# ChangUk/RecommenderSystems

Hardware: AMD Instinct MI355X
Metric: RWR seeds/sec + achieved HBM GB/s on 100M-edge bipartite graph, 1/2/4/8 GPUs (higher is better)
Workload: dtype f64

## Files before the change

### recommendersystems_amd/csrc/chain_scan.hip

```cpp
#include "engine.h"
#include "pf.h"

#include <cstdlib>

namespace rwr {

template <int G> struct CsGeom {
    static constexpr int EP = (G == 1) ? 1024 : 4096;
    static constexpr int P = (G >= 16) ? 4 : 1;
    static constexpr int E = EP * P;
    static constexpr int R = EP / 256;
    static constexpr int CH = E / G;
};
__device__ __forceinline__ int cs_pad(int q) { return q + (q >> 4); }
__device__ __forceinline__ double cs_term(const double *termp, const double *zt, const int32_t *srcp, int32_t l, int G)
{
    return zt ? zt[(size_t)srcp[l] * G] : termp[l];
}

__global__ __launch_bounds__(256) void k_cs_links(int nchunks, int CH, const int64_t *__restrict__ in_ptr,
                                                  const int32_t *__restrict__ in_src,
                                                  const int32_t *__restrict__ seeds, int32_t *__restrict__ lnk)
{
    const int slot = blockIdx.y;
// ... 288 lines not shown
{
    const int slot = blockIdx.x, lane = threadIdx.x;
    const int tile = slot / G, k = slot % G;
    const int32_t sd = seeds[slot];
    if (sd < 0) return;
    const size_t base = (size_t)slot * nchunks;
    double s = 0.0;
    unsigned redo = 0;
    if (direct) {
        for (int c = 0; c < nchunks; ++c)
            s = cs_redo_block<G>(s, n, nchunks, c, tile, k, dangling, X, seeds, c1, in_ptr, in_src, evoff, evterm, lnk);
        if (lane == 0) {
            if (sums) sums[slot] = s;
            else Y[(size_t)tile * (size_t)n * G + (size_t)sd * G + k] = s;
            if (zout) { const double rw = c1 * s; zout[(size_t)tile * (size_t)n * G + (size_t)sd * G + k] = rw * w_src[sd]; }
            if (nz_out && s != 0.0)
                atomicOr(&nz_out[(size_t)tile * (((size_t)n + 31) / 32) + ((uint32_t)sd >> 5)], 1u << (sd & 31));
        }
        return;
    }
    double ap, apn = 0.0;
    int32_t ep, epn = 0;
    long long f0, f1, f0n = 0, f1n = 0;
#define CS_LOAD(C, AP, EP, F0, F1)                                   \
    {                                                                \
        const int cc__ = (C) + lane;                                 \
        const bool v__ = cc__ < nchunks;                             \
        const size_t i__ = base + (v__ ? cc__ : nchunks - 1);        \
        AP = v__ ? approx[i__] : 0.0;                                \
        EP = e_pred[i__];                                            \
        F0 = d0[i__];                                                \
        F1 = d1[i__];                                                \
// ... 29 lines not shown
        const int L = __builtin_ctzll(bad);
        if (L > 0 && normal) s = cs_from_m(eb, __shfl(M, L - 1, WAVE));
        s = cs_redo_block<G>(s, n, nchunks, c + L, tile, k, dangling, X, seeds, c1, in_ptr, in_src, evoff, evterm, lnk);
        ++redo;
        done = L + 1;
        if (done >= WAVE || c + done >= nchunks) {
            c += WAVE;
            done = 0;
            ap = apn; ep = epn; f0 = f0n; f1 = f1n;
        }
    }
#undef CS_LOAD
    if (lane == 0) {
        if (sums) sums[slot] = s;
        else Y[(size_t)tile * (size_t)n * G + (size_t)sd * G + k] = s;
        if (nz_out && s != 0.0)
            atomicOr(&nz_out[(size_t)tile * (((size_t)n + 31) / 32) + ((uint32_t)sd >> 5)], 1u << (sd & 31));
        if (redo_count && redo) atomicAdd(redo_count, (unsigned long long)redo);
    }
}

constexpr int CS_PLAIN = 0, CS_SPLIT = 1, CS_EXACT = 2, CS_REDO = 3, CS_SPLIT2 = 4;
#ifdef RWR_EXPERIMENTS
__device__ int cs_carry_dbg = 0;
#endif
constexpr int CS_KIND_SHIFT = 12;
constexpr int CS_SIDE_WORDS = 32;
constexpr int CS_MX_LINKS = 8192;
constexpr int CS_RUN_ADDENDS = 8;
typedef double v2d_t __attribute__((ext_vector_type(2)));

__global__ __launch_bounds__(256, 6) void k_cs_block1(int32_t n, int nchunks, const uint8_t *__restrict__ dangling,
// ... 730 lines not shown
```

### recommendersystems_amd/csrc/common.h

```cpp
#pragma once
#include <hip/hip_runtime.h>
#include <stdint.h>
#include <stdio.h>
#include <string>
#include <vector>

#include "../../include/rwr.h"

namespace rwr {

void set_error(const char *fmt, ...);

#define RWR_HIP(call)                                                                         \
    do {                                                                                      \
        hipError_t e__ = (call);                                                              \
        if (e__ != hipSuccess) {                                                              \
            rwr::set_error("%s failed: %s (%s:%d)", #call, hipGetErrorString(e__), __FILE__,  \
                           __LINE__);                                                         \
            return (e__ == hipErrorOutOfMemory) ? RWR_E_NOMEM : RWR_E_HIP;                    \
        }                                                                                     \
    } while (0)

#define RWR_TRY(call)                  \
    do {                               \
// ... 11 lines not shown

static inline unsigned cdiv(size_t a, size_t b) { return (unsigned)((a + b - 1) / b); }

__host__ __device__ static inline uint64_t f64_orderable(double x)
{
    x = x + 0.0;
    uint64_t u;
    __builtin_memcpy(&u, &x, 8);
    return (u & 0x8000000000000000ull) ? ~u : (u | 0x8000000000000000ull);
}
__host__ __device__ static inline uint64_t i64_orderable(int64_t x)
{
    return (uint64_t)x ^ 0x8000000000000000ull;
}

void *pool_alloc(size_t bytes, size_t *got);
void pool_free(void *p, size_t got);

template <typename T>
struct DevBuf {
    T *p = nullptr;
    size_t count = 0;
    size_t reserved = 0;
    int32_t alloc(size_t n_elems)
    {
        release();
        if (n_elems == 0) n_elems = 1;
        p = (T *)pool_alloc(n_elems * sizeof(T), &reserved);
        if (!p) {
            const hipError_t e = hipGetLastError();
// ... 31 lines not shown
```

### recommendersystems_amd/csrc/iterate.hip

```cpp
#include "engine.h"
#include "step_plan.h"

#include <algorithm>
#include <chrono>
#include <climits>
#include <cstdlib>
#include <new>
#include <type_traits>

namespace rwr {

template <int G, bool VF>
__global__ __launch_bounds__(256) void k_spmm(int32_t n, const int64_t *__restrict__ in_ptr,
                                              const int32_t *__restrict__ in_src,
                                              const double *__restrict__ in_w,
                                              const int32_t *__restrict__ row_order, int32_t nrows,
                                              const double *__restrict__ X, double *__restrict__ Y,
                                              const int32_t *__restrict__ seeds, double c1, int skip_seed_row,
                                              const double *__restrict__ w_src, double *__restrict__ Zout)
{
    constexpr int RPW = WAVE / G;
    constexpr int U = 4;
    const int tile = blockIdx.y;
    const size_t toff = (size_t)tile * (size_t)n * G;
// ... 56 lines not shown
                                                  const int32_t *__restrict__ row_order, int32_t nrows,
                                                  const double *__restrict__ X, double *__restrict__ Y,
                                                  const int32_t *__restrict__ seeds, double c1,
                                                  int skip_seed_row, const uint32_t *__restrict__ nz_in,
                                                  uint32_t *__restrict__ nz_out,
                                                  const uint32_t *__restrict__ act,
                                                  const double *__restrict__ w_src, double *__restrict__ Zout)
{
    static_assert(G >= 8 && G <= 64, "chunked SpMM needs 8 <= G <= 64");
    constexpr int RPW = WAVE / G;
    const int tile = blockIdx.y;
    const size_t toff = (size_t)tile * (size_t)n * G;
    X += toff;
    Y += toff;
    if (VF && Zout) Zout += toff;
    const size_t nzw = ((size_t)n + 31) / 32;
    if (CHECK) nz_in += (size_t)tile * nzw;
    if (WRITE) nz_out += (size_t)tile * nzw;
    if (CHECK && act) act += (size_t)tile * nzw;
    const int lane = threadIdx.x & (WAVE - 1);
    const int sub = lane / G, k = lane % G;
    const int gbase = (lane - k) << 2;
    const int32_t my_seed = skip_seed_row ? seeds[tile * G + k] : -1;
    const int wpb = blockDim.x / WAVE;
    const int64_t nwaves = (int64_t)gridDim.x * wpb;
    for (int64_t rb = ((int64_t)blockIdx.x * wpb + threadIdx.x / WAVE) * RPW; rb < nrows; rb += nwaves * RPW) {
        const int64_t r = rb + sub;
        int32_t j = -1;
        int64_t p = 0, e = 0;
        if (r < nrows) {
            j = row_order[r];
            p = in_ptr[j];
            e = in_ptr[j + 1];
            if (CHECK && act && !((act[(uint32_t)j >> 5] >> (j & 31)) & 1u)) e = p;
        }
        double acc = 0.0;
        while (__any(p < e)) {
            const int64_t left = e - p;
            const int cnt = left > CH ? CH : (left > 0 ? (int)left : 0);
            int32_t my_idx = 0;
            double my_w = 0.0;
            if (k < cnt) {
                my_idx = in_src[p + k];
                if (!VF) my_w = in_w[p + k];
                if (CHECK) {
                    const uint32_t wd = nz_in[(uint32_t)my_idx >> 5];
                    if (!((wd >> (my_idx & 31)) & 1u)) my_idx |= (int32_t)0x80000000;
                }
            }
            const int wlo = __double2loint(my_w), whi = __double2hiint(my_w);
            if (CHECK) {
                const unsigned long long lm = __ballot(k < cnt && my_idx >= 0);
                unsigned long long um = lm;
                if (G < 64) {
#pragma unroll
                    for (int sh = G; sh < 64; sh <<= 1) um |= um >> sh;
                    um &= (1ull << (G & 63)) - 1ull;
                }
                if (__popcll(um) <= 4) {
                    while (um) {
                        const int t = __builtin_ctzll(um);
                        um &= um - 1;
                        const int idx = __builtin_amdgcn_ds_bpermute(gbase + (t << 2), my_idx);
                        if (VF) {
                            if (t < cnt && idx >= 0) acc += X[(size_t)idx * G + k];
                        } else {
                            const int lo = __builtin_amdgcn_ds_bpermute(gbase + (t << 2), wlo);
                            const int hi = __builtin_amdgcn_ds_bpermute(gbase + (t << 2), whi);
                            if (t < cnt && idx >= 0) {
                                const double rw = c1 * X[(size_t)idx * G + k];
                                acc += rw * __hiloint2double(hi, lo);
                            }
                        }
                    }
                    p += cnt;
                    continue;
                }
            }
            double xv[CH], wv[CH];
#pragma unroll
            for (int t = 0; t < CH; ++t) {
                const int idx = __builtin_amdgcn_ds_bpermute(gbase + (t << 2), my_idx);
                if (!VF) {
                    const int lo = __builtin_amdgcn_ds_bpermute(gbase + (t << 2), wlo);
                    const int hi = __builtin_amdgcn_ds_bpermute(gbase + (t << 2), whi);
                    wv[t] = __hiloint2double(hi, lo);
                }
                xv[t] = (t < cnt && idx >= 0) ? X[(size_t)idx * G + k] : 0.0;
            }
#pragma unroll
            for (int t = 0; t < CH; ++t) {
                if (t < cnt) {
                    if (VF) {
                        acc += xv[t];
                    } else {
                        double rw = c1 * xv[t];
                        acc += rw * wv[t];
                    }
                }
            }
            p += cnt;
        }
        if (j >= 0 && j != my_seed) {
            Y[(size_t)j * G + k] = acc;
            if (VF && Zout) { const double rw = c1 * acc; Zout[(size_t)j * G + k] = rw * w_src[j]; }
        }
        if (WRITE) {
            const unsigned long long nzb = __ballot(acc != 0.0);
            const unsigned long long gmask = (G == 64) ? ~0ull : (((1ull << (G & 63)) - 1ull) << (sub * G));
            if (k == 0 && j >= 0 && (nzb & gmask)) atomicOr(&nz_out[(uint32_t)j >> 5], 1u << (j & 31));
        }
    }
}

template <int G, int CH, bool CHECK, bool WRITE, bool VF, bool LIST>
__global__ __launch_bounds__(256) void k_spmm_chunked(int32_t n, const int64_t *__restrict__ in_ptr,
                                                      const int32_t *__restrict__ in_src,
                                                      const double *__restrict__ in_w,
                                                      const int32_t *__restrict__ row_order, int32_t nrows,
                                                      const double *__restrict__ X, double *__restrict__ Y,
                                                      const int32_t *__restrict__ seeds, double c1,
                                                      int skip_seed_row, const uint32_t *__restrict__ nz_in,
                                                      uint32_t *__restrict__ nz_out,
                                                      const uint32_t *__restrict__ act,
                                                      const double *__restrict__ w_src, double *__restrict__ Zout)
// ... 12 lines not shown
                                                       const int32_t *__restrict__ seeds, double c1,
                                                       int skip_seed_row, const uint32_t *__restrict__ nz_in,
                                                       uint32_t *__restrict__ nz_out,
                                                       const double *__restrict__ w_src, double *__restrict__ Zout)
{
    const int tile = blockIdx.y;
    spmm_chunked_body<G, CH, true, true, VF>(n, in_ptr, in_src, in_w, fl_rows + (size_t)tile * (size_t)n, fl_cnt[tile], X, Y,
                                             seeds, c1, skip_seed_row, nz_in, nz_out, nullptr, w_src, Zout);
}

__global__ __launch_bounds__(256) void k_mark_active(int32_t n, const uint32_t *__restrict__ nz, uint32_t *__restrict__ act,
                                                     const int64_t *__restrict__ rowptr, const int32_t *__restrict__ dst,
                                                     const uint8_t *__restrict__ etype, int G, const int32_t *__restrict__ seeds,
                                                     int32_t *__restrict__ fl_rows, int32_t *__restrict__ fl_cnt)
{
    const size_t nzw = ((size_t)n + 31) / 32;
    const int tile = blockIdx.y;
    const int lane = threadIdx.x & (WAVE - 1);
    const size_t wi = (size_t)blockIdx.x * (blockDim.x / WAVE) + threadIdx.x / WAVE;
    uint32_t *a = act + (size_t)tile * nzw;
    int32_t *list = fl_rows ? fl_rows + (size_t)tile * (size_t)n : nullptr;
    if (list && blockIdx.x == 0 && threadIdx.x < (unsigned)G) {
        const int32_t sr = seeds[tile * G + threadIdx.x];
        if (sr >= 0) {
            const uint32_t bit = 1u << (sr & 31);
            if (!(atomicOr(&a[(uint32_t)sr >> 5], bit) & bit)) list[atomicAdd(&fl_cnt[tile], 1)] = sr;
        }
    }
    if (wi >= nzw) return;
    uint32_t w = nz[(size_t)tile * nzw + wi];
    while (w) {
        const int b = __builtin_ctz(w);
        w &= w - 1;
        const int64_t i = (int64_t)wi * 32 + b;
        const int64_t p1 = rowptr[i + 1];
        if (!list) {
            for (int64_t p = rowptr[i] + lane; p < p1; p += WAVE)
                if (etype[p] != RWR_EDGE_UNDEFINED) {
                    const int32_t t = dst[p];
                    atomicOr(&a[(uint32_t)t >> 5], 1u << (t & 31));
                }
            continue;
        }
        for (int64_t p0 = rowptr[i]; p0 < p1; p0 += WAVE) {
            const int64_t p = p0 + lane;
            bool add = false;
            int32_t t = 0;
            if (p < p1 && etype[p] != RWR_EDGE_UNDEFINED) {
                t = dst[p];
// ... 50 lines not shown
            }
            acc += dg[u] ? xv[u] : (xv[u] - rw);
        }
    }
    for (; i < n; ++i) {
        double xi = x[(size_t)i * G];
        double rw = c1 * xi;
        while (nxt == i) {
            acc += rw * in_w[p];
            ++p;
            nxt = (p < e) ? in_src[p] : INT_MAX;
        }
        acc += dangling[i] ? xi : (xi - rw);
    }
    Y[(size_t)tile * (size_t)n * G + (size_t)s * G + k] = acc;
    if (nz_out && acc != 0.0)
        atomicOr(&nz_out[(size_t)tile * (((size_t)n + 31) / 32) + ((uint32_t)s >> 5)], 1u << (s & 31));
}

__global__ void k_gate(const unsigned int *__restrict__ gate, unsigned int expected)
{
    const long long t0 = __builtin_amdgcn_s_memrealtime();
    while (__hip_atomic_load(gate, __ATOMIC_RELAXED, __HIP_MEMORY_SCOPE_AGENT) < expected) {
        if (__builtin_amdgcn_s_memrealtime() - t0 > 100000) break;
        __builtin_amdgcn_s_sleep(32);
    }
}

template <int G, bool VF>
__global__ __launch_bounds__(256) void k_seed_terms(int32_t n, const int64_t *__restrict__ in_ptr,
                                                    const int32_t *__restrict__ in_src,
                                                    const double *__restrict__ in_w, const double *__restrict__ X,
                                                    const int32_t *__restrict__ seeds, double c1,
                                                    const int64_t *__restrict__ evoff, double *__restrict__ evterm,
                                                    const uint32_t *__restrict__ nz)
{
    const int slot = blockIdx.y;
    const int32_t s = seeds[slot];
    if (s < 0) return;
    const int tile = slot / G, k = slot % G;
    const double *x = X + (size_t)tile * (size_t)n * G + k;
    const int64_t p0 = in_ptr[s], deg = in_ptr[s + 1] - p0;
    double *out = evterm + evoff[slot];
    if (nz) nz += (size_t)tile * (((size_t)n + 31) / 32);
    for (int64_t q = (int64_t)blockIdx.x * blockDim.x + threadIdx.x; q < deg; q += (int64_t)gridDim.x * blockDim.x) {
        const int32_t i = in_src[p0 + q];
        if (nz && !((nz[(uint32_t)i >> 5] >> (i & 31)) & 1u)) {
            out[q] = 0.0;
        } else if (VF) {
            out[q] = x[(size_t)i * G];
        } else {
            const double rw = c1 * x[(size_t)i * G];
            out[q] = rw * in_w[p0 + q];
        }
    }
}

template <int G>
__global__ __launch_bounds__(64) void k_seed_chain_sparse(int32_t n, const int64_t *__restrict__ in_ptr,
                                                          const int32_t *__restrict__ in_src,
                                                          const uint8_t *__restrict__ dangling,
                                                          const double *__restrict__ X, double *__restrict__ Y,
                                                          const int32_t *__restrict__ seeds, double c1,
                                                          const int64_t *__restrict__ evoff,
                                                          const double *__restrict__ evterm,
                                                          const uint32_t *__restrict__ nz_x, uint32_t *__restrict__ nz_out,
                                                          unsigned int *__restrict__ gate)
{
    if (threadIdx.x == 0 && gate) __hip_atomic_fetch_add(gate, 1u, __ATOMIC_RELAXED, __HIP_MEMORY_SCOPE_AGENT);
    const int tile = blockIdx.x, lane = threadIdx.x;
    const size_t nzw = ((size_t)n + 31) / 32;
    const uint32_t *bits = nz_x + (size_t)tile * nzw;
    const double *x = X + (size_t)tile * (size_t)n * G;
    const bool consumer = lane < G;
    const int k = lane % G;
    int32_t s = -1;
    int64_t p = 0, e = 0;
    const double *termp = evterm;
    if (consumer) {
        s = seeds[tile * G + k];
        if (s >= 0) {
            p = in_ptr[s];
            e = in_ptr[s + 1];
            termp = evterm + evoff[tile * G + k] - p;
        }
    }
    double acc = 0.0;
    for (size_t w0 = 0; w0 < nzw; w0 += WAVE) {
        const uint32_t word = (w0 + lane < nzw) ? bits[w0 + lane] : 0u;
        unsigned long long mask = __ballot(word != 0u);
        while (mask) {
            const int l = __builtin_ctzll(mask);
            mask &= mask - 1;
            uint32_t wv = (uint32_t)__builtin_amdgcn_readlane((int)word, l);
            while (wv) {
                const int b = __builtin_ctz(wv);
                wv &= wv - 1;
                const int32_t i = (int32_t)((w0 + l) * 32 + b);
                if (consumer && s >= 0) {
                    while (p < e && in_src[p] < i) ++p;
                    while (p < e && in_src[p] == i) { acc += termp[p]; ++p; }
                    const double xi = x[(size_t)i * G + k];
                    const double rw = c1 * xi;
                    acc += dangling[i] ? xi : (xi - rw);
                }
            }
        }
    }
    if (consumer && s >= 0) {
        Y[(size_t)tile * (size_t)n * G + (size_t)s * G + k] = acc;
        if (nz_out && acc != 0.0)
            atomicOr(&nz_out[(size_t)tile * nzw + ((uint32_t)s >> 5)], 1u << (s & 31));
    }
}

constexpr int CH3_NSW = 6;
constexpr int CH3_NST = CH3_NSW * WAVE;
constexpr int CH3_LPT = 16;
constexpr int CH3_CE = CH3_NST * CH3_LPT;
template <int G>
__global__ __launch_bounds__(WAVE + CH3_NST) void k_seed_chain_roles(
    int32_t n, const int64_t *__restrict__ in_ptr, const int32_t *__restrict__ in_src,
    const uint8_t *__restrict__ dangling, const double *__restrict__ X, double *__restrict__ Y,
    const int32_t *__restrict__ seeds, double c1, const int64_t *__restrict__ evoff,
    const double *__restrict__ evterm, uint32_t *__restrict__ nz_out, unsigned int *__restrict__ gate)
{
    if (threadIdx.x == 0 && gate) __hip_atomic_fetch_add(gate, 1u, __ATOMIC_RELAXED, __HIP_MEMORY_SCOPE_AGENT);
// ... 105 lines not shown
        CH3_READ(ra, 0)
#pragma unroll 1
        for (int r0 = 0; r0 + 64 <= CR; r0 += 64) {
            CH3_READ(rb, r0 + 32)
            CH3_FOLD(ra, r0)
            if (r0 + 64 < CR) CH3_READ(ra, r0 + 64)
            CH3_FOLD(rb, r0 + 32)
        }
        if (CR % 64 != 0) CH3_FOLD(ra, CR - 32)
#undef CH3_READ
#undef CH3_FOLD
    }
    __builtin_amdgcn_s_setprio(0);
    if (consumer && s >= 0) {
        Y[(size_t)tile * (size_t)n * G + (size_t)s * G + k] = acc;
        if (nz_out && acc != 0.0)
            atomicOr(&nz_out[(size_t)tile * (((size_t)n + 31) / 32) + ((uint32_t)s >> 5)], 1u << (s & 31));
    }
}

__global__ void k_init_seeds(int32_t n, int ntiles, int G, double *__restrict__ X,
                             const int32_t *__restrict__ seeds, uint32_t *__restrict__ nz,
                             double *__restrict__ Z = nullptr, const double *__restrict__ w_src = nullptr, double c1 = 0.0)
{
    const int q = blockIdx.x * blockDim.x + threadIdx.x;
    if (q >= ntiles * G) return;
    const int32_t s = seeds[q];
    if (s < 0) return;
    const int tile = q / G;
    const size_t row = (size_t)tile * (size_t)n * G + (size_t)s * G;
    const double rw = c1 * (double)n;
    const double zs = Z ? rw * w_src[s] : 0.0;
    for (int kk = 0; kk < G; ++kk) {
        const bool mine = seeds[tile * G + kk] == s;
        X[row + kk] = mine ? (double)n : 0.0;
        if (Z) Z[row + kk] = mine ? zs : 0.0;
    }
    if (nz) atomicOr(&nz[(size_t)tile * (((size_t)n + 31) / 32) + ((uint32_t)s >> 5)], 1u << (s & 31));
}

__global__ __launch_bounds__(64) void k_exclude(int32_t n, int ntiles, int G, const int64_t *__restrict__ rowptr,
                                                const int32_t *__restrict__ dst, const uint8_t *__restrict__ etype,
                                                double *__restrict__ X, const int32_t *__restrict__ seeds)
{
    const int q = blockIdx.x;
    if (q >= ntiles * G) return;
    const int32_t s = seeds[q];
    if (s < 0) return;
    double *x = X + (size_t)(q / G) * (size_t)n * G + (q % G);
    const int64_t p1 = rowptr[s + 1];
    for (int64_t p = rowptr[s] + threadIdx.x; p < p1; p += WAVE)
        if (etype[p] == RWR_EDGE_LIKE) x[(size_t)dst[p] * G] = -1.0;
}
// ... 11 lines not shown
}
__global__ __launch_bounds__(256) void k_make_z(int64_t elems, int G, const double *__restrict__ X, double *__restrict__ Z,
                                                const double *__restrict__ w_src, double c1)
{
    const int64_t q = (int64_t)blockIdx.x * blockDim.x + threadIdx.x;
    if (q >= elems) return;
    const double rw = c1 * X[q];
    Z[q] = rw * w_src[q / G];
}

__global__ __launch_bounds__(256) void k_make_z_nz(int32_t lo, int32_t hi, int G, const double *__restrict__ X, double *__restrict__ Zs,
                                                   const double *__restrict__ w_src, double c1, uint32_t *__restrict__ nz)
{
    const int64_t j = ((int64_t)lo & ~(int64_t)63) + (int64_t)blockIdx.x * blockDim.x + threadIdx.x;
    bool any = false;
    if (j >= lo && j < hi) {
        const double w = w_src[j];
        const size_t at = (size_t)(j - lo) * G;
        for (int k = 0; k < G; ++k) {
            const double xv = X[(size_t)j * G + k];
            const double rw = c1 * xv;
            Zs[at + k] = rw * w;
            any = any || xv != 0.0;
        }
    }
    const unsigned long long m = __ballot(any);
    const int lane = threadIdx.x & (WAVE - 1);
    if (lane == 0 && (uint32_t)m) nz[(uint64_t)j >> 5] = (uint32_t)m;
    if (lane == 32 && (uint32_t)(m >> 32)) nz[(uint64_t)j >> 5] = (uint32_t)(m >> 32);
}


static PlanInput read_plan_knobs()
{
    PlanInput v;
    const char *e;
    if ((e = getenv("RWR_SPMM"))) v.spmm = atoi(e);
    if ((e = RWR_TUNE_ENV("RWR_NZ_ITERS"))) v.nz_iters = atoi(e);
    if ((e = getenv("RWR_ACT_ITERS"))) v.act_iters = atoi(e);
// ... 190 lines not shown
        : g(g_), G(G_), tg(tg_), d_seeds(seeds), d_evoff(evoff), c1(1 - d) ,
          X(g_->X.p), Y(g_->Y.p), Zc(g_->vf ? g_->Z0.p : nullptr), Zn(g_->vf ? g_->Z1.p : nullptr) {}

    int32_t init(bool fresh = true, bool ranks_nonneg = true, bool ranking_only = false)
    {
        const int32_t n = g->n;
        hipStream_t s = g->stream;
        const size_t elems = (size_t)tg * (size_t)n * G;
        PlanInput in = plan_knobs();
        in.n = n; in.nnz = g->nnz; in.nonneg = g->nonneg; in.big_n = spmv_big_n(); in.seed_row_kernel = g->opts.seed_row_kernel;
        in.scan_self = chain_scan_self_contained(G); in.G = G; in.tg = tg; in.c1 = c1;
        in.fresh = fresh; in.ranks_nonneg = ranks_nonneg; in.ranking_only = ranking_only;
        cfg = plan_config(in);
        if (fresh) RWR_HIP(hipMemsetAsync(X, 0, elems * sizeof(double), s));
        if (!fresh && Zc) hipLaunchKernelGGL(k_make_z, dim3(cdiv(elems, 256)), dim3(256), 0, s, (int64_t)elems, G, X, Zc, g->w_src.p, c1);
        const size_t nzw = ((size_t)n + 31) / 32;
        if (cfg.flist && g->fl_rows.ensure((size_t)tg * (size_t)n + (size_t)tg) != RWR_OK) {
            (void)hipGetLastError();
            cfg.flist = false;
        }
        if (fresh && Zc && !cfg.flist) RWR_HIP(hipMemsetAsync(Zc, 0, elems * sizeof(double), s));
        nz_cur = cfg.nz_iters > 0 ? g->d_nz.p : nullptr;
        nz_oth = cfg.nz_iters > 0 ? g->d_nz.p + (size_t)tg * nzw : nullptr;
        if (nz_cur) RWR_HIP(hipMemsetAsync(nz_cur, 0, (size_t)tg * nzw * sizeof(uint32_t), s));
        if (fresh) hipLaunchKernelGGL(k_init_seeds, dim3(cdiv((size_t)tg * G, 64)), dim3(64), 0, s, n, tg, G, X, d_seeds, nz_cur, Zc, g->w_src.p, c1);
        RWR_HIP(hipGetLastError());
        if (cfg.scan) RWR_TRY(chain_scan_prepare(g, G, tg, d_seeds, s));
        if (Zc && G == 1 && tg == 1 && cfg.addends_nonneg) RWR_TRY(sweep_prepare(g));
        if (Zc && cfg.chain_kind == 0 && !cfg.scan) RWR_TRY(ensure_in_w(g));
        return RWR_OK;
    }

    int32_t step(const StepPlan &p, Profile &prof)
    {
        const int32_t n = g->n;
        hipStream_t s = g->stream;
        const size_t nzw = ((size_t)n + 31) / 32;
        constexpr int GATE_SLOTS = 64;
        const uint32_t *nz_in = p.probe ? nz_cur : nullptr;
        uint32_t *nz_out = p.write_bits ? nz_oth : nullptr;
        if (nz_out) RWR_HIP(hipMemsetAsync(nz_out, 0, (size_t)tg * nzw * sizeof(uint32_t), s));
        uint32_t *act = p.mark ? g->d_nz.p + 2 * (size_t)tg * nzw : nullptr;
        const bool listed = p.rows.kind == Rows::Frontier;
        if (act) {
            int32_t *fl_rows = listed ? g->fl_rows.p : nullptr, *fl_cnt = listed ? fl_rows + (size_t)tg * (size_t)n : nullptr;
            RWR_HIP(hipMemsetAsync(act, 0, (size_t)tg * nzw * sizeof(uint32_t), s));
            if (fl_cnt) RWR_HIP(hipMemsetAsync(fl_cnt, 0, (size_t)tg * sizeof(int32_t), s));
            hipLaunchKernelGGL(k_mark_active, dim3(cdiv(nzw, 4), tg), dim3(256), 0, s, n, nz_in, act, g->rowptr.p,
                               g->dst.p, g->etype.p, G, d_seeds, fl_rows, fl_cnt);
        }
        const uint32_t *nz_terms = p.terms_nz ? nz_in : nullptr;
        double *zout = (Zc && p.form_z) ? Zn : nullptr;
        hipStream_t sc = p.chain_side ? g->stream2 : s;
        unsigned int *gate_it = p.gate ? g->d_gate.p + (it % GATE_SLOTS) : nullptr;
        if (p.chain != Chain::None) {
            if (!p.scan()) RWR_DISPATCH_G(G, launch_seed_terms<GG>(g, tg, X, d_seeds, c1, d_evoff, s, Zc, nz_terms));
            if (gate_it) RWR_HIP(hipMemsetAsync(gate_it, 0, sizeof(unsigned int), s));
            if (p.chain_side) { RWR_HIP(hipEventRecord(g->ev_fork, s)); RWR_HIP(hipStreamWaitEvent(sc, g->ev_fork, 0)); }
            if (p.scan() && !(p.chain_self && Zc)) RWR_DISPATCH_G(G, launch_seed_terms<GG>(g, tg, X, d_seeds, c1, d_evoff, sc, Zc, nz_terms));
            hipEvent_t c0; RWR_TRY(prof.record(c0, sc));
            if (p.scan())
                RWR_TRY(chain_scan_step(g, G, tg, X, Y, d_seeds, d_evoff, c1, nz_out, sc, p.chain_self ? Zc : nullptr,
                                        p.chain_self ? zout : nullptr));
// ... 55 lines not shown
    const size_t per_tile = mats * n * (size_t)G * sizeof(double);
    int TG = g->opts.tile_group > 0 ? g->opts.tile_group : (int)(cap / (per_tile ? per_tile : 1));
    if (TG < 1) TG = 1;
    if (TG > ntiles) TG = ntiles;
    if (TG > 65535 / G) TG = 65535 / G;
    if (g->opts.tile_group <= 0 && TG > 192) TG = 192;
    for (;;) {
        int32_t rc = g->X.ensure((size_t)TG * n * G);
        if (rc == RWR_OK) rc = g->Y.ensure((size_t)TG * n * G);
        if (rc == RWR_OK && g->vf) {
            rc = g->Z0.ensure((size_t)TG * n * G);
            if (rc == RWR_OK) rc = g->Z1.ensure((size_t)TG * n * G);
        }
        if (rc == RWR_OK && extra_mats) rc = g->cs_diff.ensure((size_t)TG * n * G);
        if (rc == RWR_OK) rc = g->d_seeds.ensure((size_t)ntiles * G);
        if (rc == RWR_OK) rc = g->d_nz.ensure(3 * (size_t)TG * ((n + 31) / 32));
        if (rc == RWR_OK) rc = g->d_gate.ensure(64);
        if (rc == RWR_OK) break;
        if (rc != RWR_E_NOMEM || TG <= 1 || g->opts.tile_group > 0) return rc;
        (void)hipGetLastError();
        g->X.release(); g->Y.release(); g->Z0.release(); g->Z1.release(); g->d_nz.release();
        if (extra_mats) g->cs_diff.release();
        TG = (TG + 1) / 2;
    }
    *TG_out = TG;
    return RWR_OK;
}

static int32_t upload_seed_slots(rwr_graph *g, const int32_t *seeds, int32_t K, int G, std::vector<int32_t> *slot_k_out,
                                 std::vector<int32_t> *slot_seed_out = nullptr)
{
// ... 558 lines not shown

int32_t part_begin(rwr_graph *g, int32_t lo, int32_t hi, const int32_t *seeds, int32_t K, double d, double *x,
                   int32_t *G_out)
{
    const int32_t n = g->n;
    if (lo < 0 || hi > n || lo > hi) { set_error("rwr_part_begin: bad slab [%d, %d)", lo, hi); return RWR_E_RANGE; }
    if (K < 1 || K > 64) { set_error("rwr_part_begin: K must be 1..64 in row-partitioned mode"); return RWR_E_UNSUPPORTED; }
    for (int32_t k = 0; k < K; ++k)
        if (seeds[k] < 0 || seeds[k] >= n) { set_error("seed %d is outside [0, %d)", seeds[k], n); return RWR_E_RANGE; }
    int G = 1;
    while (G < K) G <<= 1;
    if (g->vf) RWR_TRY(g->Z0.ensure((size_t)(hi - lo > 0 ? hi - lo : 1) * (size_t)G));
    else RWR_TRY(ensure_in_w(g));
    g->part_lo = lo; g->part_hi = hi; g->part_G = G; g->part_K = K; g->part_c1 = 1 - d;
    g->part_steps = 0;
    if (g->vf && g->nonneg && G >= 8) RWR_TRY(g->d_nz.ensure(2 * (((size_t)n + 31) / 32)));
    g->part_seeds.assign((size_t)G, -1);
    for (int32_t k = 0; k < K; ++k) g->part_seeds[k] = seeds[k];
    RWR_TRY(g->d_seeds.ensure(G));
    RWR_TRY(g->d_part.ensure((size_t)RP_GRID * G + G));
    RWR_HIP(hipMemcpy(g->d_seeds.p, g->part_seeds.data(), G * sizeof(int32_t), hipMemcpyHostToDevice));
    hipStream_t s = g->stream;
    RWR_HIP(hipMemsetAsync(x, 0, (size_t)n * G * sizeof(double), s));
    hipLaunchKernelGGL(k_init_seeds, dim3(1), dim3(64), 0, s, n, 1, G, x, g->d_seeds.p, (uint32_t *)nullptr);
    RWR_HIP(hipGetLastError());
    RWR_HIP(hipStreamSynchronize(s));
    if (G_out) *G_out = G;
    return RWR_OK;
}

static int32_t part_spmm(rwr_graph *g, const double *x, double *y, hipStream_t s)
{
    const int G = g->part_G;
    const double c1 = g->part_c1;
    if (g->vf) {
        const int64_t rows = (int64_t)g->part_hi - g->part_lo;
        if (rows > 0 && (!g->Z0.p || g->Z0.count < (size_t)rows * G)) { set_error("rwr_part_step: call rwr_part_begin"); return RWR_E_INVALID; }
        const int64_t elems = rows * G;
        const double *zin = g->Z0.p - (size_t)g->part_lo * G;
        static const int part_act_env = [] { const char *e = RWR_TUNE_ENV("RWR_PART_ACT_STEPS"); return e ? atoi(e) : 2; }();
        static const int part_nz_env = [] { const char *e = RWR_TUNE_ENV("RWR_PART_NZ_STEPS"); return e ? atoi(e) : 4; }();
        const size_t nzw = ((size_t)g->n + 31) / 32;
        const bool frontier = g->part_steps < part_nz_env && g->nonneg && G >= 8 && rows > 0 && g->d_nz.p && g->d_nz.count >= 2 * nzw;
        const bool mark = frontier && g->part_steps < part_act_env;
        ++g->part_steps;
        if (frontier) {
            uint32_t *nz = g->d_nz.p, *act = g->d_nz.p + nzw;
            RWR_HIP(hipMemsetAsync(nz, 0, (mark ? 2 : 1) * nzw * sizeof(uint32_t), s));
            const int64_t first = (int64_t)g->part_lo & ~(int64_t)63;
            hipLaunchKernelGGL(k_make_z_nz, dim3(cdiv((size_t)((int64_t)g->part_hi - first), 256)), dim3(256), 0, s, g->part_lo, g->part_hi, G, x,
                               g->Z0.p, g->w_src.p, c1, nz);
            if (mark) hipLaunchKernelGGL(k_mark_active, dim3(cdiv(nzw, 4), 1), dim3(256), 0, s, g->n, nz, act, g->rowptr.p, g->dst.p, g->etype.p,
                                         0, nullptr, nullptr, nullptr);
            RWR_DISPATCH_G(G, launch_spmm<GG>(g, 1, x, y, g->d_seeds.p, c1, 0, nz, nullptr, s, mark ? act : nullptr, zin, nullptr, false));
            return RWR_OK;
        }
        if (elems > 0)
            hipLaunchKernelGGL(k_make_z, dim3(cdiv((size_t)elems, 256)), dim3(256), 0, s, elems, G, x + (size_t)g->part_lo * G, g->Z0.p,
                               g->w_src.p + g->part_lo, c1);
        RWR_DISPATCH_G(G, launch_spmm<GG>(g, 1, x, y, g->d_seeds.p, c1, 0, nullptr, nullptr, s, nullptr, zin, nullptr, false));
    } else {
        if (!g->in_w.p) { set_error("rwr_part_step: call rwr_part_begin"); return RWR_E_INVALID; }
        RWR_DISPATCH_G(G, launch_spmm<GG>(g, 1, x, y, g->d_seeds.p, c1, 0, nullptr, nullptr, s));
    }
    return RWR_OK;
}

int32_t part_local_step(rwr_graph *g, const double *x, double *y, double *r)
// ... 77 lines not shown
```

### recommendersystems_amd/csrc/step_plan.h

```cpp
#pragma once

#include <cstdint>

namespace rwr {

struct PlanInput {
    int spmm = 1, nz_iters = 4, act_iters = -1, frontier_list = 1, chain = 1;
    int64_t act_min_n = 200000; double scan_work = 10000.0;
    int scan_side = 1, gate = 1, tail_rows = 1;
    bool two_streams = true;
    int32_t n = 0, big_n = 2000000;
    int64_t nnz = 0; bool nonneg = true;
    int seed_row_kernel = 0;
    bool scan_self = false;
    int G = 1, tg = 1;
    double c1 = 0.85;
    bool fresh = true;
    bool ranks_nonneg = true;
    bool ranking_only = false;
};

struct PlanConfig {
    int G = 1, tg = 1; bool fresh = true;
    int nz_iters = 0;
    int act_iters = 0;
    bool flist = false;
    bool addends_nonneg = false;
    bool scan = false;
    int chain_kind = 1;
    bool scan_side = false, scan_self = false;
    bool two_streams = true, gate = true;
    bool tails = false; int tail_depth = 0;
    unsigned need = 0;
};

inline PlanConfig plan_config(const PlanInput &in)
{
    PlanConfig c;
    c.G = in.G, c.tg = in.tg, c.fresh = in.fresh;
    const bool single = in.G == 1 && in.tg == 1;
    c.nz_iters = (in.G >= 8 && in.spmm != 0 && in.nonneg) ? in.nz_iters : 0;
    c.act_iters = in.act_iters >= 0 ? in.act_iters : ((in.nnz / (in.n > 0 ? in.n : 1)) <= 64 ? 2 : 1);
    if (single && in.act_iters < 0 && c.act_iters == 2 && in.n >= in.big_n) c.act_iters = 3;
    if (single && in.spmm != 0 && in.nonneg) c.nz_iters = c.act_iters;
    if (single && in.act_iters < 0 && in.n < in.act_min_n) c.nz_iters = c.act_iters = 0;
    if (!in.fresh) c.nz_iters = c.act_iters = 0;
    c.flist = in.ranking_only && in.fresh && in.frontier_list != 0 && in.G >= 8 && c.nz_iters >= 2 && c.act_iters >= 1;
    c.chain_kind = in.seed_row_kernel == 1 ? 3 : in.seed_row_kernel == 2 ? 2 : in.seed_row_kernel == 3 ? 0 : in.chain;
    const double per_seed = 0.89 * (double)in.nnz / (double)(in.n > 0 ? in.n : 1) + 6.7;
    c.addends_nonneg = in.c1 >= 0.0 && in.c1 <= 1.0 && in.nonneg && in.ranks_nonneg;
    c.scan = c.addends_nonneg && (c.chain_kind == 2 || (c.chain_kind == 1 && (double)in.tg * in.G * per_seed < in.scan_work));
    c.scan_side = in.scan_side != 0 && single && in.two_streams && in.n >= 100000;
    c.scan_self = in.scan_self, c.two_streams = in.two_streams, c.gate = in.gate != 0;
    c.tails = in.ranking_only && in.tail_rows != 0 && !single;
    return c;
}
// ... 53 lines not shown
```

Baseline: 772.7.

## Track nonzero frontier bits per 16-seed line instead of per row

Replaces the one-bit-per-row nonzero bitmap with a multi-bit-per-row bitmap for G>16, one bit per group of 16 seed columns. The SpMM gather then skips X loads for 16-lane groups whose seeds have not yet reached a source row, rather than loading whenever any seed in the tile has. This costs a larger bitmap, extra mask arithmetic in the inner loop, and an index-width limit that disables the frontier path for large n. Frontier consumers (mark_active, sparse chain) collapse the lines back to per-row bits.

```diff
diff --git a/recommendersystems_amd/csrc/chain_scan.hip b/recommendersystems_amd/csrc/chain_scan.hip
--- a/recommendersystems_amd/csrc/chain_scan.hip
+++ b/recommendersystems_amd/csrc/chain_scan.hip
@@ -326,8 +326,7 @@
             if (sums) sums[slot] = s;
             else Y[(size_t)tile * (size_t)n * G + (size_t)sd * G + k] = s;
             if (zout) { const double rw = c1 * s; zout[(size_t)tile * (size_t)n * G + (size_t)sd * G + k] = rw * w_src[sd]; }
-            if (nz_out && s != 0.0)
-                atomicOr(&nz_out[(size_t)tile * (((size_t)n + 31) / 32) + ((uint32_t)sd >> 5)], 1u << (sd & 31));
+            if (nz_out && s != 0.0) nz_set_lines(nz_out + (size_t)tile * nz_words(n, G), sd, G, nz_slot_line(k, G));
         }
         return;
     }
@@ -387,8 +386,7 @@
     if (lane == 0) {
         if (sums) sums[slot] = s;
         else Y[(size_t)tile * (size_t)n * G + (size_t)sd * G + k] = s;
-        if (nz_out && s != 0.0)
-            atomicOr(&nz_out[(size_t)tile * (((size_t)n + 31) / 32) + ((uint32_t)sd >> 5)], 1u << (sd & 31));
+        if (nz_out && s != 0.0) nz_set_lines(nz_out + (size_t)tile * nz_words(n, G), sd, G, nz_slot_line(k, G));
         if (redo_count && redo) atomicAdd(redo_count, (unsigned long long)redo);
     }
 }
diff --git a/recommendersystems_amd/csrc/common.h b/recommendersystems_amd/csrc/common.h
--- a/recommendersystems_amd/csrc/common.h
+++ b/recommendersystems_amd/csrc/common.h
@@ -49,6 +49,26 @@
     return (uint64_t)x ^ 0x8000000000000000ull;
 }
 
+__host__ __device__ constexpr int nz_lines(int G) { return G > 16 ? G / 16 : 1; }
+__host__ __device__ inline size_t nz_words(int32_t n, int G) { return ((size_t)n * nz_lines(G) + 31) / 32; }
+__host__ __device__ constexpr uint32_t nz_slot_line(int k, int G) { return 1u << (G > 16 ? k / 16 : 0); }
+__device__ inline uint32_t nz_row_lines(const uint32_t *bits, int32_t j, int G)
+{
+    const size_t b = (size_t)(uint32_t)j * nz_lines(G);
+    return (bits[b >> 5] >> (b & 31)) & ((1u << nz_lines(G)) - 1u);
+}
+__device__ inline void nz_set_lines(uint32_t *bits, int32_t j, int G, uint32_t lines)
+{
+    const size_t b = (size_t)(uint32_t)j * nz_lines(G);
+    atomicOr(&bits[b >> 5], lines << (b & 31));
+}
+__device__ inline uint32_t nz_word_rows(uint32_t w, int G)
+{
+    const int L = nz_lines(G);
+    for (int sh = 1; sh < L; sh <<= 1) w |= w >> sh;
+    return L == 1 ? w : L == 2 ? (w & 0x55555555u) : (w & 0x11111111u);
+}
+
 void *pool_alloc(size_t bytes, size_t *got);
 void pool_free(void *p, size_t got);
 
diff --git a/recommendersystems_amd/csrc/iterate.hip b/recommendersystems_amd/csrc/iterate.hip
--- a/recommendersystems_amd/csrc/iterate.hip
+++ b/recommendersystems_amd/csrc/iterate.hip
@@ -94,13 +94,16 @@
     X += toff;
     Y += toff;
     if (VF && Zout) Zout += toff;
-    const size_t nzw = ((size_t)n + 31) / 32;
-    if (CHECK) nz_in += (size_t)tile * nzw;
-    if (WRITE) nz_out += (size_t)tile * nzw;
+    const size_t nzl = nz_words(n, G), nzw = ((size_t)n + 31) / 32;
+    if (CHECK) nz_in += (size_t)tile * nzl;
+    if (WRITE) nz_out += (size_t)tile * nzl;
     if (CHECK && act) act += (size_t)tile * nzw;
     const int lane = threadIdx.x & (WAVE - 1);
     const int sub = lane / G, k = lane % G;
     const int gbase = (lane - k) << 2;
+    constexpr int L = nz_lines(G), IB = 31 - L;
+    constexpr int32_t IDX = L > 1 ? (int32_t)((1u << IB) - 1u) : (int32_t)0x7fffffff;
+    const int32_t dead = (int32_t)(0x80000000u | (L > 1 ? 1u << (IB + k / 16) : 0u));
     const int32_t my_seed = skip_seed_row ? seeds[tile * G + k] : -1;
     const int wpb = blockDim.x / WAVE;
     const int64_t nwaves = (int64_t)gridDim.x * wpb;
@@ -124,8 +127,9 @@
                 my_idx = in_src[p + k];
                 if (!VF) my_w = in_w[p + k];
                 if (CHECK) {
-                    const uint32_t wd = nz_in[(uint32_t)my_idx >> 5];
-                    if (!((wd >> (my_idx & 31)) & 1u)) my_idx |= (int32_t)0x80000000;
+                    const uint32_t lv = nz_row_lines(nz_in, my_idx, G);
+                    if (!lv) my_idx |= (int32_t)0x80000000;
+                    else if (L > 1) my_idx |= (int32_t)((~lv & ((1u << L) - 1u)) << IB);
                 }
             }
             const int wlo = __double2loint(my_w), whi = __double2hiint(my_w);
@@ -143,12 +147,12 @@
                         um &= um - 1;
                         const int idx = __builtin_amdgcn_ds_bpermute(gbase + (t << 2), my_idx);
                         if (VF) {
-                            if (t < cnt && idx >= 0) acc += X[(size_t)idx * G + k];
+                            if (t < cnt && !(idx & dead)) acc += X[(size_t)(idx & IDX) * G + k];
                         } else {
                             const int lo = __builtin_amdgcn_ds_bpermute(gbase + (t << 2), wlo);
                             const int hi = __builtin_amdgcn_ds_bpermute(gbase + (t << 2), whi);
-                            if (t < cnt && idx >= 0) {
-                                const double rw = c1 * X[(size_t)idx * G + k];
+                            if (t < cnt && !(idx & dead)) {
+                                const double rw = c1 * X[(size_t)(idx & IDX) * G + k];
                                 acc += rw * __hiloint2double(hi, lo);
                             }
                         }
@@ -166,7 +170,8 @@
                     const int hi = __builtin_amdgcn_ds_bpermute(gbase + (t << 2), whi);
                     wv[t] = __hiloint2double(hi, lo);
                 }
-                xv[t] = (t < cnt && idx >= 0) ? X[(size_t)idx * G + k] : 0.0;
+                if (CHECK) xv[t] = (t < cnt && !(idx & dead)) ? X[(size_t)(idx & IDX) * G + k] : 0.0;
+                else xv[t] = (t < cnt && idx >= 0) ? X[(size_t)idx * G + k] : 0.0;
             }
 #pragma unroll
             for (int t = 0; t < CH; ++t) {
@@ -186,9 +191,12 @@
             if (VF && Zout) { const double rw = c1 * acc; Zout[(size_t)j * G + k] = rw * w_src[j]; }
         }
         if (WRITE) {
-            const unsigned long long nzb = __ballot(acc != 0.0);
-            const unsigned long long gmask = (G == 64) ? ~0ull : (((1ull << (G & 63)) - 1ull) << (sub * G));
-            if (k == 0 && j >= 0 && (nzb & gmask)) atomicOr(&nz_out[(uint32_t)j >> 5], 1u << (j & 31));
+            const unsigned long long nzb = __ballot(acc != 0.0) >> (sub * G);
+            uint32_t lines = 0;
+#pragma unroll
+            for (int l = 0; l < L; ++l)
+                if ((nzb >> (16 * l)) & (G >= 16 ? 0xffffull : (1ull << G) - 1ull)) lines |= 1u << l;
+            if (k == 0 && j >= 0 && lines) nz_set_lines(nz_out, j, G, lines);
         }
     }
 }
@@ -231,7 +239,8 @@
                                                      const uint8_t *__restrict__ etype, int G, const int32_t *__restrict__ seeds,
                                                      int32_t *__restrict__ fl_rows, int32_t *__restrict__ fl_cnt)
 {
-    const size_t nzw = ((size_t)n + 31) / 32;
+    const size_t nzw = ((size_t)n + 31) / 32, nzl = nz_words(n, G);
+    const int L = nz_lines(G);
     const int tile = blockIdx.y;
     const int lane = threadIdx.x & (WAVE - 1);
     const size_t wi = (size_t)blockIdx.x * (blockDim.x / WAVE) + threadIdx.x / WAVE;
@@ -244,12 +253,12 @@
             if (!(atomicOr(&a[(uint32_t)sr >> 5], bit) & bit)) list[atomicAdd(&fl_cnt[tile], 1)] = sr;
         }
     }
-    if (wi >= nzw) return;
-    uint32_t w = nz[(size_t)tile * nzw + wi];
+    if (wi >= nzl) return;
+    uint32_t w = nz_word_rows(nz[(size_t)tile * nzl + wi], G);
     while (w) {
         const int b = __builtin_ctz(w);
         w &= w - 1;
-        const int64_t i = (int64_t)wi * 32 + b;
+        const int64_t i = ((int64_t)wi * 32 + b) / L;
         const int64_t p1 = rowptr[i + 1];
         if (!list) {
             for (int64_t p = rowptr[i] + lane; p < p1; p += WAVE)
@@ -330,8 +339,7 @@
         acc += dangling[i] ? xi : (xi - rw);
     }
     Y[(size_t)tile * (size_t)n * G + (size_t)s * G + k] = acc;
-    if (nz_out && acc != 0.0)
-        atomicOr(&nz_out[(size_t)tile * (((size_t)n + 31) / 32) + ((uint32_t)s >> 5)], 1u << (s & 31));
+    if (nz_out && acc != 0.0) nz_set_lines(nz_out + (size_t)tile * nz_words(n, G), s, G, nz_slot_line(k, G));
 }
 
 __global__ void k_gate(const unsigned int *__restrict__ gate, unsigned int expected)
@@ -358,10 +366,10 @@
     const double *x = X + (size_t)tile * (size_t)n * G + k;
     const int64_t p0 = in_ptr[s], deg = in_ptr[s + 1] - p0;
     double *out = evterm + evoff[slot];
-    if (nz) nz += (size_t)tile * (((size_t)n + 31) / 32);
+    if (nz) nz += (size_t)tile * nz_words(n, G);
     for (int64_t q = (int64_t)blockIdx.x * blockDim.x + threadIdx.x; q < deg; q += (int64_t)gridDim.x * blockDim.x) {
         const int32_t i = in_src[p0 + q];
-        if (nz && !((nz[(uint32_t)i >> 5] >> (i & 31)) & 1u)) {
+        if (nz && !(nz_row_lines(nz, i, G) & nz_slot_line(k, G))) {
             out[q] = 0.0;
         } else if (VF) {
             out[q] = x[(size_t)i * G];
@@ -385,7 +393,8 @@
 {
     if (threadIdx.x == 0 && gate) __hip_atomic_fetch_add(gate, 1u, __ATOMIC_RELAXED, __HIP_MEMORY_SCOPE_AGENT);
     const int tile = blockIdx.x, lane = threadIdx.x;
-    const size_t nzw = ((size_t)n + 31) / 32;
+    const size_t nzw = nz_words(n, G);
+    constexpr int L = nz_lines(G);
     const uint32_t *bits = nz_x + (size_t)tile * nzw;
     const double *x = X + (size_t)tile * (size_t)n * G;
     const bool consumer = lane < G;
@@ -403,7 +412,7 @@
     }
     double acc = 0.0;
     for (size_t w0 = 0; w0 < nzw; w0 += WAVE) {
-        const uint32_t word = (w0 + lane < nzw) ? bits[w0 + lane] : 0u;
+        const uint32_t word = (w0 + lane < nzw) ? nz_word_rows(bits[w0 + lane], G) : 0u;
         unsigned long long mask = __ballot(word != 0u);
         while (mask) {
             const int l = __builtin_ctzll(mask);
@@ -412,7 +421,7 @@
             while (wv) {
                 const int b = __builtin_ctz(wv);
                 wv &= wv - 1;
-                const int32_t i = (int32_t)((w0 + l) * 32 + b);
+                const int32_t i = (int32_t)(((w0 + l) * 32 + b) / L);
                 if (consumer && s >= 0) {
                     while (p < e && in_src[p] < i) ++p;
                     while (p < e && in_src[p] == i) { acc += termp[p]; ++p; }
@@ -425,8 +434,7 @@
     }
     if (consumer && s >= 0) {
         Y[(size_t)tile * (size_t)n * G + (size_t)s * G + k] = acc;
-        if (nz_out && acc != 0.0)
-            atomicOr(&nz_out[(size_t)tile * nzw + ((uint32_t)s >> 5)], 1u << (s & 31));
+        if (nz_out && acc != 0.0) nz_set_lines(nz_out + (size_t)tile * nzw, s, G, nz_slot_line(k, G));
     }
 }
 
@@ -562,8 +570,7 @@
     __builtin_amdgcn_s_setprio(0);
     if (consumer && s >= 0) {
         Y[(size_t)tile * (size_t)n * G + (size_t)s * G + k] = acc;
-        if (nz_out && acc != 0.0)
-            atomicOr(&nz_out[(size_t)tile * (((size_t)n + 31) / 32) + ((uint32_t)s >> 5)], 1u << (s & 31));
+        if (nz_out && acc != 0.0) nz_set_lines(nz_out + (size_t)tile * nz_words(n, G), s, G, nz_slot_line(k, G));
     }
 }
 
@@ -584,7 +591,7 @@
         X[row + kk] = mine ? (double)n : 0.0;
         if (Z) Z[row + kk] = mine ? zs : 0.0;
     }
-    if (nz) atomicOr(&nz[(size_t)tile * (((size_t)n + 31) / 32) + ((uint32_t)s >> 5)], 1u << (s & 31));
+    if (nz) nz_set_lines(nz + (size_t)tile * nz_words(n, G), s, G, nz_slot_line(q % G, G));
 }
 
 __global__ __launch_bounds__(64) void k_exclude(int32_t n, int ntiles, int G, const int64_t *__restrict__ rowptr,
@@ -626,6 +633,7 @@
 {
     const int64_t j = ((int64_t)lo & ~(int64_t)63) + (int64_t)blockIdx.x * blockDim.x + threadIdx.x;
     bool any = false;
+    uint32_t lines = 0;
     if (j >= lo && j < hi) {
         const double w = w_src[j];
         const size_t at = (size_t)(j - lo) * G;
@@ -634,7 +642,12 @@
             const double rw = c1 * xv;
             Zs[at + k] = rw * w;
             any = any || xv != 0.0;
-        }
+            if (xv != 0.0) lines |= nz_slot_line(k, G);
+        }
+    }
+    if (nz_lines(G) > 1) {
+        if (lines) nz_set_lines(nz, (int32_t)j, G, lines);
+        return;
     }
     const unsigned long long m = __ballot(any);
     const int lane = threadIdx.x & (WAVE - 1);
@@ -855,15 +868,15 @@
         cfg = plan_config(in);
         if (fresh) RWR_HIP(hipMemsetAsync(X, 0, elems * sizeof(double), s));
         if (!fresh && Zc) hipLaunchKernelGGL(k_make_z, dim3(cdiv(elems, 256)), dim3(256), 0, s, (int64_t)elems, G, X, Zc, g->w_src.p, c1);
-        const size_t nzw = ((size_t)n + 31) / 32;
+        const size_t nzl = nz_words(n, G);
         if (cfg.flist && g->fl_rows.ensure((size_t)tg * (size_t)n + (size_t)tg) != RWR_OK) {
             (void)hipGetLastError();
             cfg.flist = false;
         }
         if (fresh && Zc && !cfg.flist) RWR_HIP(hipMemsetAsync(Zc, 0, elems * sizeof(double), s));
         nz_cur = cfg.nz_iters > 0 ? g->d_nz.p : nullptr;
-        nz_oth = cfg.nz_iters > 0 ? g->d_nz.p + (size_t)tg * nzw : nullptr;
-        if (nz_cur) RWR_HIP(hipMemsetAsync(nz_cur, 0, (size_t)tg * nzw * sizeof(uint32_t), s));
+        nz_oth = cfg.nz_iters > 0 ? g->d_nz.p + (size_t)tg * nzl : nullptr;
+        if (nz_cur) RWR_HIP(hipMemsetAsync(nz_cur, 0, (size_t)tg * nzl * sizeof(uint32_t), s));
         if (fresh) hipLaunchKernelGGL(k_init_seeds, dim3(cdiv((size_t)tg * G, 64)), dim3(64), 0, s, n, tg, G, X, d_seeds, nz_cur, Zc, g->w_src.p, c1);
         RWR_HIP(hipGetLastError());
         if (cfg.scan) RWR_TRY(chain_scan_prepare(g, G, tg, d_seeds, s));
@@ -876,18 +889,18 @@
     {
         const int32_t n = g->n;
         hipStream_t s = g->stream;
-        const size_t nzw = ((size_t)n + 31) / 32;
+        const size_t nzw = ((size_t)n + 31) / 32, nzl = nz_words(n, G);
         constexpr int GATE_SLOTS = 64;
         const uint32_t *nz_in = p.probe ? nz_cur : nullptr;
         uint32_t *nz_out = p.write_bits ? nz_oth : nullptr;
-        if (nz_out) RWR_HIP(hipMemsetAsync(nz_out, 0, (size_t)tg * nzw * sizeof(uint32_t), s));
-        uint32_t *act = p.mark ? g->d_nz.p + 2 * (size_t)tg * nzw : nullptr;
+        if (nz_out) RWR_HIP(hipMemsetAsync(nz_out, 0, (size_t)tg * nzl * sizeof(uint32_t), s));
+        uint32_t *act = p.mark ? g->d_nz.p + 2 * (size_t)tg * nzl : nullptr;
         const bool listed = p.rows.kind == Rows::Frontier;
         if (act) {
             int32_t *fl_rows = listed ? g->fl_rows.p : nullptr, *fl_cnt = listed ? fl_rows + (size_t)tg * (size_t)n : nullptr;
             RWR_HIP(hipMemsetAsync(act, 0, (size_t)tg * nzw * sizeof(uint32_t), s));
             if (fl_cnt) RWR_HIP(hipMemsetAsync(fl_cnt, 0, (size_t)tg * sizeof(int32_t), s));
-            hipLaunchKernelGGL(k_mark_active, dim3(cdiv(nzw, 4), tg), dim3(256), 0, s, n, nz_in, act, g->rowptr.p,
+            hipLaunchKernelGGL(k_mark_active, dim3(cdiv(nzl, 4), tg), dim3(256), 0, s, n, nz_in, act, g->rowptr.p,
                                g->dst.p, g->etype.p, G, d_seeds, fl_rows, fl_cnt);
         }
         const uint32_t *nz_terms = p.terms_nz ? nz_in : nullptr;
@@ -973,7 +986,7 @@
         }
         if (rc == RWR_OK && extra_mats) rc = g->cs_diff.ensure((size_t)TG * n * G);
         if (rc == RWR_OK) rc = g->d_seeds.ensure((size_t)ntiles * G);
-        if (rc == RWR_OK) rc = g->d_nz.ensure(3 * (size_t)TG * ((n + 31) / 32));
+        if (rc == RWR_OK) rc = g->d_nz.ensure(2 * (size_t)TG * nz_words(n, G) + (size_t)TG * ((n + 31) / 32));
         if (rc == RWR_OK) rc = g->d_gate.ensure(64);
         if (rc == RWR_OK) break;
         if (rc != RWR_E_NOMEM || TG <= 1 || g->opts.tile_group > 0) return rc;
@@ -1562,7 +1575,7 @@
     else RWR_TRY(ensure_in_w(g));
     g->part_lo = lo; g->part_hi = hi; g->part_G = G; g->part_K = K; g->part_c1 = 1 - d;
     g->part_steps = 0;
-    if (g->vf && g->nonneg && G >= 8) RWR_TRY(g->d_nz.ensure(2 * (((size_t)n + 31) / 32)));
+    if (g->vf && g->nonneg && G >= 8) RWR_TRY(g->d_nz.ensure(nz_words(n, G) + ((size_t)n + 31) / 32));
     g->part_seeds.assign((size_t)G, -1);
     for (int32_t k = 0; k < K; ++k) g->part_seeds[k] = seeds[k];
     RWR_TRY(g->d_seeds.ensure(G));
@@ -1588,18 +1601,19 @@
         const double *zin = g->Z0.p - (size_t)g->part_lo * G;
         static const int part_act_env = [] { const char *e = RWR_TUNE_ENV("RWR_PART_ACT_STEPS"); return e ? atoi(e) : 2; }();
         static const int part_nz_env = [] { const char *e = RWR_TUNE_ENV("RWR_PART_NZ_STEPS"); return e ? atoi(e) : 4; }();
-        const size_t nzw = ((size_t)g->n + 31) / 32;
-        const bool frontier = g->part_steps < part_nz_env && g->nonneg && G >= 8 && rows > 0 && g->d_nz.p && g->d_nz.count >= 2 * nzw;
+        const size_t nzw = ((size_t)g->n + 31) / 32, nzl = nz_words(g->n, G);
+        const bool frontier = g->part_steps < part_nz_env && g->nonneg && G >= 8 && nz_index_fits(g->n, G) && rows > 0 && g->d_nz.p &&
+                              g->d_nz.count >= nzl + nzw;
         const bool mark = frontier && g->part_steps < part_act_env;
         ++g->part_steps;
         if (frontier) {
-            uint32_t *nz = g->d_nz.p, *act = g->d_nz.p + nzw;
-            RWR_HIP(hipMemsetAsync(nz, 0, (mark ? 2 : 1) * nzw * sizeof(uint32_t), s));
+            uint32_t *nz = g->d_nz.p, *act = g->d_nz.p + nzl;
+            RWR_HIP(hipMemsetAsync(nz, 0, (nzl + (mark ? nzw : 0)) * sizeof(uint32_t), s));
             const int64_t first = (int64_t)g->part_lo & ~(int64_t)63;
             hipLaunchKernelGGL(k_make_z_nz, dim3(cdiv((size_t)((int64_t)g->part_hi - first), 256)), dim3(256), 0, s, g->part_lo, g->part_hi, G, x,
                                g->Z0.p, g->w_src.p, c1, nz);
-            if (mark) hipLaunchKernelGGL(k_mark_active, dim3(cdiv(nzw, 4), 1), dim3(256), 0, s, g->n, nz, act, g->rowptr.p, g->dst.p, g->etype.p,
-                                         0, nullptr, nullptr, nullptr);
+            if (mark) hipLaunchKernelGGL(k_mark_active, dim3(cdiv(nzl, 4), 1), dim3(256), 0, s, g->n, nz, act, g->rowptr.p, g->dst.p, g->etype.p,
+                                         G, nullptr, nullptr, nullptr);
             RWR_DISPATCH_G(G, launch_spmm<GG>(g, 1, x, y, g->d_seeds.p, c1, 0, nz, nullptr, s, mark ? act : nullptr, zin, nullptr, false));
             return RWR_OK;
         }
diff --git a/recommendersystems_amd/csrc/step_plan.h b/recommendersystems_amd/csrc/step_plan.h
--- a/recommendersystems_amd/csrc/step_plan.h
+++ b/recommendersystems_amd/csrc/step_plan.h
@@ -34,12 +34,14 @@
     unsigned need = 0;
 };
 
+inline bool nz_index_fits(int64_t n, int G) { return G <= 16 || n <= ((int64_t)1 << (31 - G / 16)); }
+
 inline PlanConfig plan_config(const PlanInput &in)
 {
     PlanConfig c;
     c.G = in.G, c.tg = in.tg, c.fresh = in.fresh;
     const bool single = in.G == 1 && in.tg == 1;
-    c.nz_iters = (in.G >= 8 && in.spmm != 0 && in.nonneg) ? in.nz_iters : 0;
+    c.nz_iters = (in.G >= 8 && in.spmm != 0 && in.nonneg && nz_index_fits(in.n, in.G)) ? in.nz_iters : 0;
     c.act_iters = in.act_iters >= 0 ? in.act_iters : ((in.nnz / (in.n > 0 ? in.n : 1)) <= 64 ? 2 : 1);
     if (single && in.act_iters < 0 && c.act_iters == 2 && in.n >= in.big_n) c.act_iters = 3;
     if (single && in.spmm != 0 && in.nonneg) c.nz_iters = c.act_iters;
```

New measurement: 782.2 (median of 6 runs). 1.2% higher.
